# grossmanlev/FL-distributed-delay

Measured on AMD Instinct MI355X. Metric: simulated worker-steps/sec (node) @1024 workers, delay 50; aggregation HBM GB/s, higher is better.
Workload: dtype f32

## Files before the change

fl-distributed-delay_amd/csrc/common.h:

```cpp
#pragma once
#include <hip/hip_runtime.h>
#include <stdint.h>
#include <stdlib.h>

#define FLSIM_WAVE 64

#if !defined(FLSIM_LAB) &&                                                                  \
    (defined(FLSIM_X6_FRESH) || defined(FLSIM_X6_PP_V) || defined(FLSIM_DG_FMS) ||          \
     defined(FLSIM_DIRECT_FENCES) || defined(FLSIM_DX6_FENCES) || defined(FLSIM_BUFLOAD) ||  \
     defined(FLSIM_SEQ_EARLY_EXIT) || defined(FLSIM_X6_FLUSH) || defined(FLSIM_WGRAD_X6) ||     \
     defined(FLSIM_ZL1F) || defined(FLSIM_SINGLE_BUF) || defined(FLSIM_DG3_FM) || defined(FLSIM_DX_FM))
#error "FLSIM_* measurement overrides need a lab build (make LAB=1)"
#endif

typedef float f32x4 __attribute__((ext_vector_type(4)));

namespace flsim {

void set_error(const char* fmt, ...);
const char* last_error();

#define FLSIM_CHECK_HIP(expr)                                                           \
    do {                                                                                \
        hipError_t _e = (expr);                                                         \
        if (_e != hipSuccess) {                                                         \
            ::flsim::set_error("%s failed: %s (%s:%d)", #expr, hipGetErrorString(_e),   \
// ... 72 lines not shown
```

fl-distributed-delay_amd/csrc/epi_xs.h:

```cpp
#pragma once
#include "loaders.h"
#include "split.h"

namespace flsim {

__device__ __forceinline__ f32x4 mask4(f32x4 t, uint32_t pos) {
    return f32x4{(pos & 1) ? t.x : 0.f, (pos & 2) ? t.y : 0.f, (pos & 4) ? t.z : 0.f,
                 (pos & 8) ? t.w : 0.f};
}

template <int NC, int AHW>
__device__ __forceinline__ void mask_tile_sm(float* tile, int ld, const float* act, int m0, int rows,
                                             int n0, int n4, int tid, int nt) {
    const f32x2* a2 = reinterpret_cast<const f32x2*>(act);
    for (int s = 0; 4 * s < n4; ++s) {
        for (int q = tid; q < rows * 4; q += nt) {
            const int r = q >> 2, c = 4 * s + (q & 3);
            const f32x2 a = a2[2 * xs_unit<NC, AHW, true>((unsigned)(m0 + r), n0 / 4 + c)];
            f32x4* t = reinterpret_cast<f32x4*>(tile + r * ld + 4 * c);
            *t = mask4(*t, xs_pos4(a));
        }
    }
    __syncthreads();
}

template <int NC, bool SM = false, int HW = 1>
struct EpiBiasReluXs {
    static constexpr bool ASUM = false;
    static constexpr bool STAGED = true;
    static constexpr bool PARTIAL = true;
    static constexpr int NCOL = NC;
    float* Yhm;
    float* Yl;
    const float* bias;
    int M;
    float* Yf = nullptr;
    __device__ float value(int, float v) const { return v; }
    __device__ void store_rows(const float* tile, int ld, int m0, int bm, int n0, int bn, int tid,
                               int nt) const {
        const int rows = M - m0 < bm ? M - m0 : bm;
        const int n4 = bn / 4;
        for (int q = tid; q < rows * n4; q += nt) {
            const int r = q / n4, c = q - r * n4;
            const f32x4 t = *reinterpret_cast<const f32x4*>(tile + r * ld + 4 * c);
            const f32x4 b = *reinterpret_cast<const f32x4*>(bias + n0 + 4 * c);
            const f32x4 v = {fmaxf(t.x + b.x, 0.f), fmaxf(t.y + b.y, 0.f), fmaxf(t.z + b.z, 0.f),
                             fmaxf(t.w + b.w, 0.f)};
            xs_store_f(Yhm, Yl, Yf, xs_unit<NC, HW, SM>((unsigned)(m0 + r), n0 / 4 + c), v);
        }
    }
};

template <int NC, bool OUT_XS, bool ASM = false, int AHW = 1>
struct EpiMaskXs {
    static constexpr bool ASUM = false;
    static constexpr bool STAGED = true;
    static constexpr bool PARTIAL = true;
    static constexpr int NCOL = NC;
    float* Y;
    float* Yl;
    const float* act;
    int M;
    static constexpr int BATCH = 8;
// ... 106 lines not shown
        for (int pos = 0; pos < 4; ++pos) {
            f32x4 o;
            o.x = (id & 0xffu) == (uint32_t)pos ? g.x : 0.f;
            o.y = ((id >> 8) & 0xffu) == (uint32_t)pos ? g.y : 0.f;
            o.z = ((id >> 16) & 0xffu) == (uint32_t)pos ? g.z : 0.f;
            o.w = (id >> 24) == (uint32_t)pos ? g.w : 0.f;
            const long u = u0 + ((pos >> 1) * (2 * PW) + (pos & 1)) * (long)N4;
            if constexpr (OUT_XS)
                xs_store(dZhm, dZl, u, o);
            else
                st_nt4(dZhm + 4 * u, o);
        }
    }
};

template <int PH, int PW, int C, bool SM = false>
struct EpiPoolDropXs {
    static constexpr bool ASUM = false;
    static constexpr bool STAGED = true;
    static constexpr int NCOL = C;
    float* dhm;
    float* dl;
    uint8_t* idx;
    const float* bias;
    const WorkerRec* workers;
    uint64_t seed;
    uint32_t site, thr;
    float scale;
    int dropout;
    int M;
    float* df = nullptr;
    __device__ float value(int, float v) const { return v; }
    __device__ void store_rows(const float* tile, int ld, int m0, int bm, int tid, int nt) const {
        const int rows = M - m0 < bm ? M - m0 : bm;
        constexpr int C4 = C / 4;
        const int total = rows / 4 * C4;
        for (int u = tid; u < total; u += nt) {
            const int pl = u / C4, c = u - pl * C4;
            const f32x4 b = *reinterpret_cast<const f32x4*>(bias + 4 * c);
            f32x4 x[4];
#pragma unroll
            for (int r = 0; r < 4; ++r) {
                const f32x4 t = *reinterpret_cast<const f32x4*>(tile + (4 * pl + r) * ld + 4 * c);
                x[r] = f32x4{fmaxf(t.x + b.x, 0.f), fmaxf(t.y + b.y, 0.f), fmaxf(t.z + b.z, 0.f),
                             fmaxf(t.w + b.w, 0.f)};
            }
            const int q = (m0 >> 2) + pl;
            const int pw = q % PW;
            const int ph = (q / PW) % PH;
            const int s = q / (PW * PH);
            f32x4 out;
            uint32_t id = 0;
#pragma unroll
            for (int e = 0; e < 4; ++e) {
                float mv = x[0][e];
                int mi = 0;
#pragma unroll
                for (int r = 1; r < 4; ++r)
                    if (x[r][e] > mv) { mv = x[r][e]; mi = r; }
                float o = mv;
                if (dropout) {
                    const int w = s / SAMPLES_PER_WORKER;
// ... 17 lines not shown
```

fl-distributed-delay_amd/csrc/gemm_core.h:

```cpp
#pragma once
#include <type_traits>

#include "common.h"

namespace flsim {

constexpr int GK = 16;

__device__ __forceinline__ int kc_swz(int row) { return (4 - ((row >> 2) & 3)) & 3; }

template <int ROWS>
struct KCTile {
    static constexpr int FLOATS = ROWS * GK;
    __device__ static inline int chunk_off(int row, int chunk) {
        return row * GK + 4 * (chunk ^ kc_swz(row));
    }
};
template <int ROWS>
struct KMTile {
    static constexpr int STRIDE = ROWS + 4;
    static constexpr int DUMMY = GK * STRIDE;
    static constexpr int FLOATS = GK * STRIDE + 4;
};

// ... 57 lines not shown
    if constexpr (IsPartial<EPI>::value)
        epi.store_rows(tile, ld, m0, bm, n0, bn, tid, nt);
    else
        epi.store_rows(tile, ld, m0, bm, tid, nt);
}

template <class E, class = void>
struct HasPre : std::false_type {};
template <class E>
struct HasPre<E, std::void_t<decltype(E::PRE)>> : std::bool_constant<E::PRE> {};

template <class L, class = void>
struct WantsN0 : std::false_type {};
template <class L>
struct WantsN0<L, std::void_t<decltype(L::WANTS_N0)>> : std::bool_constant<L::WANTS_N0> {};

template <class E, class = void>
struct HasBiasRing : std::false_type {};
template <class E>
struct HasBiasRing<E, std::void_t<decltype(E::BIAS_RING)>> : std::bool_constant<E::BIAS_RING> {};

#ifndef FLSIM_SINGLE_BUF
#define FLSIM_SINGLE_BUF 2
#endif

template <int FM, int FN, int WAVES_M, int WAVES_N, class AL, class BL, class EPI>
__global__ void __launch_bounds__(64 * WAVES_M * WAVES_N)
gemm_kernel(AL al, BL bl, EPI epi, int ksteps_total, int ksteps_per_split, int tiles_m,
            int tiles_n) {
    constexpr int BM = 16 * FM * WAVES_M;
// ... 166 lines not shown
```

fl-distributed-delay_amd/csrc/gemm_direct.h:

```cpp
#pragma once
#include "loaders.h"

namespace flsim {

#ifndef FLSIM_DIRECT_FENCES
#define FLSIM_DIRECT_FENCES 1
#endif
constexpr bool DIRECT_FENCES = FLSIM_DIRECT_FENCES;

template <int IH, int IW, int CI, int PAD, int FM, bool WIN = false, int OHX = 0,
          class SRC = BufSrc>
struct Im2colDirect {
    using Unit = typename SRC::Unit;
    static constexpr int PIX = SRC::SM ? GK : CI;
    static constexpr int SLICE = SRC::SM ? IH * IW * GK : GK;
    static constexpr int OH = OHX > 0 ? OHX : IH + 2 * PAD - 2;
    static constexpr int OW = OHX > 0 ? OHX : IW + 2 * PAD - 2;
    static constexpr int PH = OH / 2, PW = OW / 2;
    static constexpr int ROWS_PER_IMG = WIN ? 4 * PH * PW : OH * OW;
    static_assert(CI % 16 == 0, "direct A needs whole 16-channel slices");

    const float* X;
    const float* XL = nullptr;
    int M;
    unsigned vb[FM];
    unsigned short tapmask[FM];
    SRC buf;

    __device__ void setup(int r0, int lane) {
        const int q = lane >> 4;
        buf.init(X, XL, (unsigned long)((M + ROWS_PER_IMG - 1) / ROWS_PER_IMG) * IH * IW * CI * 4);
#pragma unroll
        for (int f = 0; f < FM; ++f) {
            const int m = r0 + 16 * f + (lane & 15);
            long base = 0;
            int msk = 0;
            if (m < M) {
                const int nimg = m / ROWS_PER_IMG;
                const int rem = m - nimg * ROWS_PER_IMG;
                int oh, ow;
                if constexpr (WIN) {
                    const int qq = rem >> 2;
                    const int ph = qq / PW;
                    oh = 2 * ph + ((rem >> 1) & 1);
                    ow = 2 * (qq - ph * PW) + (rem & 1);
                } else {
                    oh = rem / OW;
                    ow = rem - oh * OW;
                }
                base = (long)nimg * IH * IW * CI + ((long)(oh - PAD) * IW + (ow - PAD)) * PIX +
                       4 * q;
#pragma unroll
                for (int t = 0; t < 9; ++t) {
                    const int ih = oh + t / 3 - PAD, iw = ow + t % 3 - PAD;
// ... 173 lines not shown
```

fl-distributed-delay_amd/csrc/gemm_dx6.h:

```cpp
#pragma once
#include "gemm_direct.h"
#include "gemm_x6.h"

namespace flsim {

#ifndef FLSIM_DX6_FENCES
#define FLSIM_DX6_FENCES 1
#endif
constexpr bool DX6_FENCES = FLSIM_DX6_FENCES;

template <int TR, int NT, int NPL>
struct RowsKCStageXs {
    using Unit = XsUnit;
    static constexpr int ROWS = TR;
    static constexpr bool KC = true;
    static constexpr int TOTAL = ROWS * 4;
    static constexpr int UNITS = (TOTAL + NT - 1) / NT;
    static constexpr int PLANE = KCTile<ROWS>::FLOATS;
    static constexpr int SPARE = NPL * PLANE;
    static constexpr int FLOATS = NPL * PLANE + 4;
    static_assert(NPL == 2 || NPL == 3, "");
    const float* P;
    const float* PL;
    long ld;
// ... 87 lines not shown
    __syncthreads();
    if constexpr (WAVES == 8) {
        if (wave >= 4) __builtin_amdgcn_s_setprio(1);
    }
    for (int s = 0; s < nst; ++s) {
        const float* Bs = lds + (s & 1) * STG;
        float* Bn = lds + ((s + 1) & 1) * STG;
        const int kn = (s + 1) * KB;
#pragma unroll
        for (int kk = 0; kk < KB; ++kk) {
            const int ks = s * KB + kk;
            if (kk > 0) bl.store(Bn + (kk - 1) * BFL, rb);
            bl.load(kn + kk, rb);
            ad.load(ks + DEPTH, ra[(kk + DEPTH) % R]);
            if constexpr (DX6_FENCES) __builtin_amdgcn_sched_barrier(0);
            const float* Bk = Bs + kk * BFL;
            f32x4 a0[FM], a1[FM];
#pragma unroll
            for (int i = 0; i < FM; ++i) {
                a0[i] = ra[kk % R][i].hm;
                a1[i] = xs_hl(ra[kk % R][i]);
            }
#pragma unroll
            for (int j = 0; j < FN; ++j) {
                const f32x4 x0 = read_frag<true, BN>(Bk, 16 * j, lane);
                const f32x4 x2 = read_frag<true, BN>(Bk + PLANE, 16 * j, lane);
                f32x4 x1;
                if constexpr (BFL >= 3 * PLANE)
                    x1 = read_frag<true, BN>(Bk + 2 * PLANE, 16 * j, lane);
                else
                    x1 = f32x4{x0.z, x0.w, x0.x, x0.y};
#pragma unroll
                for (int i = 0; i < FM; ++i) {
                    acc[i][j] = x6_step<x6_fresh(true)>(acc[i][j], a0[i], a1[i], x0, x1, x2);
                }
            }
            if constexpr (DX6_FENCES) __builtin_amdgcn_sched_barrier(0);
        }
        bl.store(Bn + (KB - 1) * BFL, rb);
        __syncthreads();
    }

    if constexpr (STAGED) {
        static_assert(BN == EPI::NCOL || (IsPartial<EPI>::value && EPI::NCOL % BN == 0),
                      "staged epilogue needs the full row in one block");
        constexpr int PASSES = (WAVES + WM_PASS - 1) / WM_PASS;
#pragma unroll 1
        for (int pass = 0; pass < PASSES; ++pass) {
            __syncthreads();
// ... 31 lines not shown
```

fl-distributed-delay_amd/csrc/gemm_x6.h:

```cpp
#pragma once
#include "gemm_core.h"
#include "split.h"

namespace flsim {

__device__ __forceinline__ f32x4 mfma_x32(f32x4 a, f32x4 b, f32x4 c) {
    return __builtin_amdgcn_mfma_f32_16x16x32_bf16(__builtin_bit_cast(bf16x8v, a),
                                                   __builtin_bit_cast(bf16x8v, b), c, 0, 0, 0);
}

template <bool FRESH>
__device__ __forceinline__ f32x4 x6_step(f32x4 acc, f32x4 a0, f32x4 a1, f32x4 b0, f32x4 b1,
                                         f32x4 b2) {
    if constexpr (FRESH) {
        f32x4 t = mfma_x32(a1, b2, f32x4{0.f, 0.f, 0.f, 0.f});
        t = mfma_x32(a0, b1, t);
        t = mfma_x32(a0, b0, t);
        return acc + t;
    } else {
        acc = mfma_x32(a1, b2, acc);
        acc = mfma_x32(a0, b1, acc);
        return mfma_x32(a0, b0, acc);
    }
}
// ... 155 lines not shown
    const int nb = gridDim.x;
    const int b = blockIdx.x;
    const int q = nb / 8, r = nb % 8, xcd = b % 8;
    const int L = (xcd < r ? xcd * (q + 1) : r * (q + 1) + (xcd - r) * q) + b / 8;
    const int tn = L % gy;
    const int tm = (L / gy) % gx;
    const int tz = L / (gx * gy);
    const int m0 = tm * BM;
    const int n0 = tn * BN;
    const int ks0 = tz * ksteps_per_split;
    int ks1 = ks0 + ksteps_per_split;
    if (ks1 > ksteps_total) ks1 = ksteps_total;

    al.setup(m0, tid);
    bl.setup(n0, tid);

    f32x4 acc[FM][FN];
#pragma unroll
    for (int i = 0; i < FM; ++i)
#pragma unroll
        for (int j = 0; j < FN; ++j) acc[i][j] = f32x4{0.f, 0.f, 0.f, 0.f};

    float asum = 0.f;
    f32x4 bacc[AMF ? FM : 1];
#pragma unroll
    for (int i = 0; i < (AMF ? FM : 1); ++i) bacc[i] = f32x4{0.f, 0.f, 0.f, 0.f};
    const bool bwave = AMF && tn == 0 && wn == 0;
    typename AL::Unit ra[AL::UNITS];
    typename BL::Unit rb[BL::UNITS];
    auto stage = [&](float* s) {
        al.each_unit(ra, [&](int a, int c, const auto& v, bool ok) { TA::store(s, a, c, v, ok); });
        bl.each_unit(rb, [&](int a, int c, const auto& v, bool ok) {
            TB::store(s + TA::FL, a, c, v, ok);
        });
    };

    if (ks0 < ks1) {
        al.load(ks0, ra);
        bl.load(ks0, rb);
        stage(lds);
        if (ks0 + 1 < ks1) {
            al.load(ks0 + 1, ra);
            bl.load(ks0 + 1, rb);
        }
    }
    __syncthreads();
    if constexpr (WAVES_M * WAVES_N == 8) {
        if (wave >= 4) __builtin_amdgcn_s_setprio(1);
    }
    int cur = 0;
    constexpr bool PP_KC = X6_PP_V > 0 && AL::KC && BL::KC && !X6Fresh<EPI>::value &&
                           std::is_same_v<typename AL::Unit, XsUnit> &&
                           std::is_same_v<typename BL::Unit, XsUnit>;
    constexpr bool PP = PP_KC;
    constexpr int PV = X6_PP_V, PW = X6_PP_W, PL = X6_PP_L;
    constexpr int FLUSH = AL::KC ? 0 : FLSIM_X6_FLUSH;
    f32x4 tot[FLUSH ? FM : 1][FLUSH ? FN : 1];
    f32x4 btot[FLUSH && AMF ? FM : 1];
    if constexpr (FLUSH > 0) {
#pragma unroll
        for (int i = 0; i < FM; ++i) {
#pragma unroll
            for (int j = 0; j < FN; ++j) tot[i][j] = f32x4{0.f, 0.f, 0.f, 0.f};
            if constexpr (AMF) btot[i] = f32x4{0.f, 0.f, 0.f, 0.f};
        }
    }
    auto main_loop = [&](auto with_sum) {
        constexpr bool WS = decltype(with_sum)::value;
        for (int ks = ks0; ks < ks1; ++ks) {
            if constexpr (PP) {
                stage(lds + (cur ^ 1) * BUF);
                const int kl = ks + 2 < ks1 ? ks + 2 : ks1 - 1;
                al.load(kl, ra);
                bl.load(kl, rb);
            } else if (ks + 1 < ks1) {
                stage(lds + (cur ^ 1) * BUF);
                if (ks + 2 < ks1) {
                    al.load(ks + 2, ra);
                    bl.load(ks + 2, rb);
                }
            }
            const float* A = lds + cur * BUF;
            const float* B = A + TA::FL;
            if constexpr (WS && !AMF) {
                if (tid < BM) asum += TA::colsum(A, tid);
            }
            typename TB::Frag bf[FN];
#pragma unroll
            for (int j = 0; j < FN; ++j) bf[j] = TB::frag(B, wn * 16 * FN + 16 * j, lane);
#pragma unroll
            for (int i = 0; i < FM; ++i) {
                const typename TA::Frag af = TA::frag(A, wm * 16 * FM + 16 * i, lane);
                if constexpr (WS && AMF) {
                    if constexpr (x6_fresh_bias()) {
// ... 119 lines not shown
```

fl-distributed-delay_amd/csrc/loaders.h:

```cpp
#pragma once
#include "gemm_core.h"
#include "pn1.h"
#include "split.h"

namespace flsim {

__device__ __forceinline__ f32x4 ldg4(const float* p) { return *reinterpret_cast<const f32x4*>(p); }
__device__ __forceinline__ f32x4 zero4() { return f32x4{0.f, 0.f, 0.f, 0.f}; }
__device__ __forceinline__ void st_nt4(float* p, f32x4 v) {
    __builtin_nontemporal_store(v, reinterpret_cast<f32x4*>(p));
}

__device__ __forceinline__ f32x4 ldg4_or0(const float* p, const float* , bool ok) {
    return ok ? ldg4(p) : zero4();
}

#ifndef FLSIM_BUFLOAD
#define FLSIM_BUFLOAD 1
#endif
constexpr unsigned BUF_OOB = 0xfffffff0u;
__device__ __forceinline__ __amdgpu_buffer_rsrc_t raw_rsrc(const void* base, unsigned long bytes) {
    const unsigned n = bytes < (unsigned long)BUF_OOB ? (unsigned)bytes : BUF_OOB;
    return __builtin_amdgcn_make_buffer_rsrc(const_cast<void*>(base), (short)0, (int)n, 0x00020000);
}
// ... 61 lines not shown
    static constexpr unsigned find(bool want_shift) {
        for (unsigned sh = 4; sh < 24; ++sh) {
            const unsigned m = ((1u << sh) + D - 1) / D;
            if ((unsigned long long)(R - 1) * m >= (1ull << 24) * 256ull) break;
            bool ok = true;
            for (unsigned r = 0; r < R && ok; ++r) ok = ((r * m) >> sh) == r / D;
            if (ok) return want_shift ? sh : m;
        }
        return 0;
    }
    static constexpr unsigned M = find(false), SH = find(true);
    static_assert(M != 0 && R * M < (1u << 31) && R < (1u << 24), "no 24-bit magic for this range");
    __device__ static unsigned div(unsigned r) { return __umul24(r, M) >> SH; }
};

template <int IH, int IW, int CI, int PAD, int TR, int NT, bool WIN = false, int OHX = 0,
          class SRC = BufSrc>
struct Im2colKC {
    using Unit = typename SRC::Unit;
    static_assert(!SRC::SM, "pixel-major operand");
    static constexpr int ROWS = TR;
    static constexpr bool KC = true;
    static constexpr int OH = OHX > 0 ? OHX : IH + 2 * PAD - 2;
    static constexpr int OW = OHX > 0 ? OHX : IW + 2 * PAD - 2;
    static constexpr int PH = OH / 2, PW = OW / 2;
    static constexpr int ROWS_PER_IMG = WIN ? 4 * PH * PW : OH * OW;
    static constexpr int TOTAL = ROWS * 4;
    static constexpr int UNITS = (TOTAL + NT - 1) / NT;
    static constexpr bool TAP_UNIFORM = CI % 16 == 0;
    static_assert(NT % 4 == 0, "");
    static_assert(CI == 4 || CI % 16 == 0, "");

    const float* X;
    const float* XL = nullptr;
    int M;
    long base[UNITS];
    unsigned vb[UNITS];
    short tapmask[UNITS];
    short row[UNITS];
    int q;
    SRC buf;
    static_assert(FLSIM_BUFLOAD || !SRC::SPLIT, "split operands use buffer loads");

    __device__ void setup(int m0, int tid) {
        q = tid & 3;
        if constexpr (FLSIM_BUFLOAD)
            buf.init(X, XL, (unsigned long)((M + ROWS_PER_IMG - 1) / ROWS_PER_IMG) * IH * IW * CI * 4);
#pragma unroll
        for (int j = 0; j < UNITS; ++j) {
            const int u = tid + j * NT;
            const int r = u >> 2;
            row[j] = (short)r;
            const int m = m0 + r;
            base[j] = 0;
            tapmask[j] = 0;
            if (u < TOTAL && m < M) {
                const int nimg = m / ROWS_PER_IMG;
                const int rem = m - nimg * ROWS_PER_IMG;
                int oh, ow;
                if constexpr (WIN) {
                    const int qq = rem >> 2;
                    const int ph = qq / PW;
                    oh = 2 * ph + ((rem >> 1) & 1);
                    ow = 2 * (qq - ph * PW) + (rem & 1);
                } else {
                    oh = rem / OW;
                    ow = rem - oh * OW;
                }
                base[j] = ((long)nimg * IH * IW + (long)(oh - PAD) * IW + (ow - PAD)) * CI + 4 * q;
                int msk = 0;
#pragma unroll
                for (int t = 0; t < 9; ++t) {
                    const int ih = oh + t / 3 - PAD, iw = ow + t % 3 - PAD;
// ... 474 lines not shown
    float* Y;
    const float* bias;
    int M;
    __device__ float value(int n, float v) const { return fmaxf(v + bias[n], 0.f); }
    __device__ void store_rows(const float* tile, int ld, int m0, int bm, int tid, int nt) const {
        const int rows = M - m0 < bm ? M - m0 : bm;
        constexpr int N4 = NC / 4;
        f32x4* dst = reinterpret_cast<f32x4*>(Y + (long)m0 * NC);
        for (int q = tid; q < rows * N4; q += nt) {
            const int r = q / N4, c = q - r * N4;
            st_nt4(reinterpret_cast<float*>(dst + q), *reinterpret_cast<const f32x4*>(tile + r * ld + 4 * c));
        }
    }
};

template <int PH, int PW, int C, bool NCHW_OUT>
struct EpiPoolDrop {
    static constexpr bool ASUM = false;
    float* d;
    uint8_t* idx;
    const float* bias;
    const WorkerRec* workers;
    uint64_t seed;
    uint32_t site, thr;
    float scale;
    int dropout;
    int M;
    __device__ void apply4(int m, int n, int z, f32x4 v) const {
        if (n >= C || m >= M) return;
        const float b = bias[n];
        float mv = fmaxf(v[0] + b, 0.f);
        int mi = 0;
#pragma unroll
        for (int r = 1; r < 4; ++r) {
            const float x = fmaxf(v[r] + b, 0.f);
            if (x > mv) { mv = x; mi = r; }
        }
        const int q = m >> 2;
        const int pw = q % PW;
        const int ph = (q / PW) % PH;
        const int s = q / (PW * PH);
        const int w = s / SAMPLES_PER_WORKER;
        const int nl = s - w * SAMPLES_PER_WORKER;
        float out = mv;
        if (dropout) {
            const WorkerRec wr = workers[w];
            const uint32_t en = (uint32_t)(((nl * C + n) * PH + ph) * PW + pw);
            out = philox_word(seed, wr.t, wr.i, site, en) >= thr ? mv * scale : 0.f;
        }
        const long e = (long)q * C + n;
        idx[e] = (uint8_t)mi;
        if (NCHW_OUT)
            d[(long)s * (C * PH * PW) + (n * PH + ph) * PW + pw] = out;
// ... 221 lines not shown
```

fl-distributed-delay_amd/csrc/net_kernels.h:

```cpp
#pragma once
#include "epi_xs.h"
#include "gemm_direct.h"
#include "gemm_dx6.h"
#include "gemm_x6.h"
#include "loaders.h"
#include "pn1.h"
#include "probe.h"

namespace flsim {

static __global__ void __launch_bounds__(256)
k_fill_batch(const uint8_t* __restrict__ pool, const int32_t* __restrict__ labels,
             const int32_t* __restrict__ list_a, int len_a, const int32_t* __restrict__ list_b,
             int len_b, const WorkerRec* __restrict__ workers, int n_workers_total, uint64_t seed,
             const float* __restrict__ lut, float* __restrict__ x0, int32_t* __restrict__ y) {
    const int s = blockIdx.x;
    const int w = s / SAMPLES_PER_WORKER;
    const int j = s - w * SAMPLES_PER_WORKER;
    const WorkerRec wr = workers[w];
    const uint32_t bsz = wr.pad ? wr.pad : (uint32_t)SAMPLES_PER_WORKER;
    const uint32_t q = (wr.i >> 20) * SAMPLES_PER_WORKER + (uint32_t)j;
    float* out = x0 + (long)s * 4096;
    if (q >= bsz) {
        if (threadIdx.x == 0) y[s] = -1;
// ... 827 lines not shown
}

template <int IH, int IW, int CI, int PAD, int FM, int FN, int WM, int WN, int FMS, int FNS,
          int WMS, int WNS, int VO = 0, bool DZC = false, bool X6 = false, class SRC = BufSrc,
          class SRCB = SRC>
static int conv_wgrad_sz(const float* dz, const float* X, int S, int CO, int KP, float* slab,
                         float* bslab, int Z, hipStream_t st, int kid, int kreal, int zinit,
                         int* zused, const float* dzl = nullptr, const float* Xl = nullptr) {
    if (S <= small_chunk_samples())
        return conv_wgrad<IH, IW, CI, PAD, FMS, FNS, WMS, WNS, VO, DZC, X6, SRC, SRCB>(
            dz, X, S, CO, KP, slab, bslab, Z, st, kid, kreal, zinit, zused, dzl, Xl);
    return conv_wgrad<IH, IW, CI, PAD, FM, FN, WM, WN, VO, DZC, X6, SRC, SRCB>(
        dz, X, S, CO, KP, slab, bslab, Z, st, kid, kreal, zinit, zused, dzl, Xl);
}

template <int IH, int IW, int CI, int PAD, int FM, int FN, int WAVES, int KB, int DEPTH, int NPL,
          bool WIN, int OHX, class ASRC = XsSrc, class EPI>
static int conv_dx6(XsT X, int S, XsT W, int N, int KP, const EPI& epi, hipStream_t st, int kid,
                    int kreal) {
    static_assert(ASRC::SPLIT, "split input");
    using AD = Im2colDirect<IH, IW, CI, PAD, FM, WIN, OHX, ASRC>;
    using BL = RowsKCStageXs<16 * FN, 64 * WAVES, NPL>;
    constexpr int BM = 16 * FM * WAVES, BN = 16 * FN;
    FLSIM_REQUIRE((KP / GK) % KB == 0, "direct GEMM: %d k-steps not a multiple of %d", KP / GK, KB);
    AD ad;
    ad.X = X.hm;
    ad.XL = X.l;
    ad.M = S * AD::ROWS_PER_IMG;
    BL bl;
    bl.P = W.hm;
    bl.PL = W.l;
    bl.ld = KP;
    bl.NR = N;
    const int tm = ceil_div(ad.M, BM), tn = ceil_div(N, BN);
    const ProbeSlot ps = probe_begin();
    hipExtLaunchKernelGGL((gemm_dx6_kernel<FM, FN, WAVES, KB, DEPTH, AD, BL, EPI>),
                          dim3(tm * tn), dim3(64 * WAVES), 0, st, ps.start, ps.stop, 0, ad, bl,
                          epi, KP / GK, tm, tn);
    FLSIM_LAUNCH_CHECK();
    return probe_end(ps, kid, 2.0 * ad.M * N * kreal);
}

template <int IH, int IW, int CI, int PAD, int FM, int FN, int WM, int WN, bool WIN, int OHX,
          class EPI>
static int conv_xs(XsT X, int S, XsT W, int N, int KP, const EPI& epi, hipStream_t st, int kid,
                   int kreal) {
    constexpr int NT = 64 * WM * WN;
    constexpr int BM = 16 * FM * WM, BN = 16 * FN * WN;
    using AL = Im2colKC<IH, IW, CI, PAD, BM, NT, WIN, OHX, XsSrc>;
    using BL = RowsKC<BN, NT, XsSrc>;
    AL al;
    al.X = X.hm;
    al.XL = X.l;
    al.M = S * AL::ROWS_PER_IMG;
    BL bl;
    bl.P = W.hm;
    bl.PL = W.l;
    bl.ld = KP;
    bl.NR = N;
    return launch_gemm<FM, FN, WM, WN, true>(al, bl, epi, al.M, N, KP / GK, 1, st, kid,
                                             2.0 * al.M * N * kreal);
}

template <int IH, int IW, int CI, int CO, int PAD, int FM, int FN, int WM, int WN, bool NCHW_OUT,
          bool X6 = false>
static int conv_pool_fwd(const float* X, int S, const float* Wpk, int KP, float* d, uint8_t* idx,
                         const float* bias, const WorkerRec* workers, uint64_t seed, uint32_t site,
                         uint32_t thr, float scale, int dropout, hipStream_t st, int kid,
                         int kreal) {
    constexpr int NT = 64 * WM * WN;
    constexpr int BM = 16 * FM * WM, BN = 16 * FN * WN;
    using AL = Im2colKC<IH, IW, CI, PAD, BM, NT, true>;
    using BL = RowsKC<BN, NT>;
    AL al;
    al.X = X;
    al.M = S * AL::ROWS_PER_IMG;
// ... 55 lines not shown
```

fl-distributed-delay_amd/csrc/pn1_net.hip:

```cpp
#include <stdarg.h>
#include <stdio.h>
#include <string.h>

#include <mutex>
#include <unordered_map>

#include "net_abi.h"

namespace flsim {

static thread_local char g_err[512];
void set_error(const char* fmt, ...) {
    va_list ap;
    va_start(ap, fmt);
    vsnprintf(g_err, sizeof(g_err), fmt, ap);
    va_end(ap);
}
const char* last_error() { return g_err; }

struct ConvGeo {
    int CI, CIP, CO, H;
    int KP;
    int ZW;
};
// ... 231 lines not shown
    const long units = M / C1_ROWS;
    const int grid = (int)(units / 4 < 2048 ? (units + 3) / 4 : 2048);
    const ProbeSlot ps = probe_begin();
    hipExtLaunchKernelGGL(k_conv1_fwd, dim3(grid), dim3(256), 0, st, ps.start, ps.stop, 0, x0, W,
                          bias, a1.hm, a1.l, a1f, units);
    FLSIM_LAUNCH_CHECK();
    return probe_end(ps, K_FWD1, 2.0 * M * 48 * 27);
}

#ifndef FLSIM_DX_FM
#define FLSIM_DX_FM 4
#endif
constexpr int DX_FM = FLSIM_DX_FM, DX_FMS = 1, DX_KB = 3, DX_DEPTH = 2, DX_NPL = 2;


template <int IH, int IW, int CI, int PAD, int FN, bool WIN, int OHX, int FM = DX_FM,
          int WAVES = 8, int FMS = (FM == DX_FM ? DX_FMS : FM / 2), class EPI>
static int dx6(XsT X, int S, XsT W, int N, int KP, const EPI& epi, hipStream_t st, int kid,
               int kreal) {
    if (S <= small_chunk_samples())
        return conv_dx6<IH, IW, CI, PAD, FMS, FN, WAVES, DX_KB, DX_DEPTH, DX_NPL, WIN, OHX,
                        XsSrcSM>(X, S, W, N, KP, epi, st, kid, kreal);
    return conv_dx6<IH, IW, CI, PAD, FM, FN, WAVES, DX_KB, DX_DEPTH, DX_NPL, WIN, OHX, XsSrcSM>(
        X, S, W, N, KP, epi, st, kid, kreal);
}

template <int IH, int IW, int CI, int PAD, int FM, int FN, int WM, int WN, bool WIN, int OHX,
          class EPI>
static int xs(XsT X, int S, XsT W, int N, int KP, const EPI& epi, hipStream_t st, int kid,
              int kreal) {
    if (S <= small_chunk_samples())
        return conv_xs<IH, IW, CI, PAD, FM / 2, FN, WM, WN, WIN, OHX>(X, S, W, N, KP, epi, st, kid,
                                                                     kreal);
    return conv_xs<IH, IW, CI, PAD, FM, FN, WM, WN, WIN, OHX>(X, S, W, N, KP, epi, st, kid, kreal);
}

static int forward(const GradState& g, const WS& w, const float* theta, int S,
                   const WorkerRec* workers, uint64_t seed, int dropout, hipStream_t st) {
    const XsT a1 = w.x(w.a1, w.a1l), d1 = w.x(w.d1, w.d1l), a3 = w.x(w.a3, w.a3l);
    const XsT d2 = w.x(w.d2, w.d2l), a5 = w.x(w.a5, w.a5l);
    RC(conv1_fwd(w.x0, theta + P_OFF[0], theta + P_OFF[1], a1, w.a1f, S, st));
    RC((dx6<34, 34, 48, 2, 3, true, 0, 4, 4, 2>(a1, S, g.wfx[1], 48, 432,
        EpiPoolDropXs<18, 18, 48, true>{d1.hm, d1.l, w.i1, theta + P_OFF[3], workers, seed, SITE_DROP1,
                                  THR_P25, SCALE_P25, dropout, S * 18 * 18 * 4, w.d1f}, st,
        K_FWD2, 432)));
    RC((dx6<18, 18, 48, 2, 6, false, 0>(d1, S, g.wfx[2], 96, 432,
        EpiBiasReluXs<96, true, 400>{a3.hm, a3.l, theta + P_OFF[5], S * 20 * 20, w.a3f}, st, K_FWD3,
        432)));
    RC((dx6<20, 20, 96, 2, 6, true, 0>(a3, S, g.wfx[3], 96, 864,
        EpiPoolDropXs<11, 11, 96>{d2.hm, d2.l, w.i2, theta + P_OFF[7], workers, seed, SITE_DROP2,
                                  THR_P25, SCALE_P25, dropout, S * 11 * 11 * 4, w.d2f}, st,
        K_FWD4, 864)));
    RC((xs<11, 11, 96, 2, 4, 6, 4, 2, false, 0>(d2, S, g.wfx[4], 192, 864,
        EpiBiasReluXs<192>{a5.hm, a5.l, theta + P_OFF[9], S * 13 * 13, w.a5f}, st, K_FWD5, 864)));
    RC((xs<13, 13, 192, 2, 4, 6, 4, 2, true, 0>(a5, S, g.wfx[5], 192, 1728,
        EpiPoolDrop<7, 7, 192, true>{w.d3, w.i3, theta + P_OFF[11], workers, seed, SITE_DROP3,
                                     THR_P25, SCALE_P25, dropout, S * 7 * 7 * 4}, st, K_FWD6,
        1728)));
    if (S <= 2048)
        RC((linear_fwd<1, 2, 2, 2, true, EpiSlabStoreFresh>(w.d3, theta + P_OFF[12], w.part, S,
                                                            512, 9408, ZL1F, st, K_L1F)));
    else if (S <= 4096)
        RC((linear_fwd<2, 2, 2, 2, true, EpiSlabStoreFresh>(w.d3, theta + P_OFF[12], w.part, S,
                                                            512, 9408, ZL1F, st, K_L1F)));
    else
        RC((linear_fwd<4, 4, 2, 2, true, EpiSlabStoreFresh>(w.d3, theta + P_OFF[12], w.part, S,
                                                            512, 9408, ZL1F, st, K_L1F)));
    RC(linear_finish(w.part, ZL1F, theta + P_OFF[13], w.e1, S, 512, workers, seed, SITE_DROP4,
                     THR_P50, SCALE_P50, dropout, st));
    RC((linear_fwd<2, 2, 2, 2>(w.e1, theta + P_OFF[14], w.part, S, 256, 512, 1, st, K_L2F)));
    RC(linear_finish(w.part, 1, theta + P_OFF[15], w.e2, S, 256, workers, seed, SITE_DROP5,
                     THR_P50, SCALE_P50, dropout, st));
    return 0;
// ... 565 lines not shown
```

Baseline: 1173.

## Reorder conv GEMM rows image-minor to skip out-of-bounds padding taps

Adds an image-minor row mapping (RowMap) so each GEMM tile or wave covers the same output pixel across a group of images. That makes the set of in-bounds 3x3 taps uniform per tile, and the k-loop can skip padding taps entirely: remapped k-steps in the x6 GEMM, predicated steps in dx6. Only the fifth forward conv layer enables it by default; the other layers get compile-time switches. Epilogues remap rows back to image-major order. The cost is extra index arithmetic, a padded M extent rounded up to whole groups, and a per-tile varying k-loop length that can unbalance work across tiles.

```diff
diff --git a/fl-distributed-delay_amd/csrc/common.h b/fl-distributed-delay_amd/csrc/common.h
--- a/fl-distributed-delay_amd/csrc/common.h
+++ b/fl-distributed-delay_amd/csrc/common.h
@@ -9,7 +9,9 @@
     (defined(FLSIM_X6_FRESH) || defined(FLSIM_X6_PP_V) || defined(FLSIM_DG_FMS) ||          \
      defined(FLSIM_DIRECT_FENCES) || defined(FLSIM_DX6_FENCES) || defined(FLSIM_BUFLOAD) ||  \
      defined(FLSIM_SEQ_EARLY_EXIT) || defined(FLSIM_X6_FLUSH) || defined(FLSIM_WGRAD_X6) ||     \
-     defined(FLSIM_ZL1F) || defined(FLSIM_SINGLE_BUF) || defined(FLSIM_DG3_FM) || defined(FLSIM_DX_FM))
+     defined(FLSIM_ZL1F) || defined(FLSIM_SINGLE_BUF) || defined(FLSIM_DG3_FM) || defined(FLSIM_DX_FM) || \
+     defined(FLSIM_FWD_IM2) || defined(FLSIM_FWD_IM3) || defined(FLSIM_FWD_IM4) ||            \
+     defined(FLSIM_FWD_IM5) || defined(FLSIM_FWD_IM6))
 #error "FLSIM_* measurement overrides need a lab build (make LAB=1)"
 #endif
 
diff --git a/fl-distributed-delay_amd/csrc/epi_xs.h b/fl-distributed-delay_amd/csrc/epi_xs.h
--- a/fl-distributed-delay_amd/csrc/epi_xs.h
+++ b/fl-distributed-delay_amd/csrc/epi_xs.h
@@ -24,7 +24,7 @@
     __syncthreads();
 }
 
-template <int NC, bool SM = false, int HW = 1>
+template <int NC, bool SM = false, int HW = 1, int GRP = 0>
 struct EpiBiasReluXs {
     static constexpr bool ASUM = false;
     static constexpr bool STAGED = true;
@@ -38,15 +38,22 @@
     __device__ float value(int, float v) const { return v; }
     __device__ void store_rows(const float* tile, int ld, int m0, int bm, int n0, int bn, int tid,
                                int nt) const {
-        const int rows = M - m0 < bm ? M - m0 : bm;
+        const int rows = GRP > 0 || M - m0 >= bm ? bm : M - m0;
         const int n4 = bn / 4;
         for (int q = tid; q < rows * n4; q += nt) {
             const int r = q / n4, c = q - r * n4;
+            unsigned m = (unsigned)(m0 + r);
+            if constexpr (GRP > 0) {
+                unsigned img, pix;
+                RowMap<GRP, HW>::split(m, img, pix);
+                if (img >= (unsigned)(M / HW)) continue;
+                m = img * (unsigned)HW + pix;
+            }
             const f32x4 t = *reinterpret_cast<const f32x4*>(tile + r * ld + 4 * c);
             const f32x4 b = *reinterpret_cast<const f32x4*>(bias + n0 + 4 * c);
             const f32x4 v = {fmaxf(t.x + b.x, 0.f), fmaxf(t.y + b.y, 0.f), fmaxf(t.z + b.z, 0.f),
                              fmaxf(t.w + b.w, 0.f)};
-            xs_store_f(Yhm, Yl, Yf, xs_unit<NC, HW, SM>((unsigned)(m0 + r), n0 / 4 + c), v);
+            xs_store_f(Yhm, Yl, Yf, xs_unit<NC, HW, SM>(m, n0 / 4 + c), v);
         }
     }
 };
@@ -183,7 +190,7 @@
     }
 };
 
-template <int PH, int PW, int C, bool SM = false>
+template <int PH, int PW, int C, bool SM = false, int GRP = 0>
 struct EpiPoolDropXs {
     static constexpr bool ASUM = false;
     static constexpr bool STAGED = true;
@@ -201,11 +208,18 @@
     float* df = nullptr;
     __device__ float value(int, float v) const { return v; }
     __device__ void store_rows(const float* tile, int ld, int m0, int bm, int tid, int nt) const {
-        const int rows = M - m0 < bm ? M - m0 : bm;
+        const int rows = GRP > 0 || M - m0 >= bm ? bm : M - m0;
         constexpr int C4 = C / 4;
         const int total = rows / 4 * C4;
         for (int u = tid; u < total; u += nt) {
             const int pl = u / C4, c = u - pl * C4;
+            int q = (m0 >> 2) + pl;
+            if constexpr (GRP > 0) {
+                unsigned img, win;
+                RowMap<GRP, PH * PW>::split((unsigned)q, img, win);
+                if (img >= (unsigned)(M / (4 * PH * PW))) continue;
+                q = (int)(img * (unsigned)(PH * PW) + win);
+            }
             const f32x4 b = *reinterpret_cast<const f32x4*>(bias + 4 * c);
             f32x4 x[4];
 #pragma unroll
@@ -214,7 +228,6 @@
                 x[r] = f32x4{fmaxf(t.x + b.x, 0.f), fmaxf(t.y + b.y, 0.f), fmaxf(t.z + b.z, 0.f),
                              fmaxf(t.w + b.w, 0.f)};
             }
-            const int q = (m0 >> 2) + pl;
             const int pw = q % PW;
             const int ph = (q / PW) % PH;
             const int s = q / (PW * PH);
diff --git a/fl-distributed-delay_amd/csrc/gemm_core.h b/fl-distributed-delay_amd/csrc/gemm_core.h
--- a/fl-distributed-delay_amd/csrc/gemm_core.h
+++ b/fl-distributed-delay_amd/csrc/gemm_core.h
@@ -95,6 +95,11 @@
 struct WantsN0 : std::false_type {};
 template <class L>
 struct WantsN0<L, std::void_t<decltype(L::WANTS_N0)>> : std::bool_constant<L::WANTS_N0> {};
+
+template <class L, class = void>
+struct TapSkip : std::false_type {};
+template <class L>
+struct TapSkip<L, std::void_t<decltype(L::TAP_SKIP)>> : std::bool_constant<L::TAP_SKIP> {};
 
 template <class E, class = void>
 struct HasBiasRing : std::false_type {};
diff --git a/fl-distributed-delay_amd/csrc/gemm_direct.h b/fl-distributed-delay_amd/csrc/gemm_direct.h
--- a/fl-distributed-delay_amd/csrc/gemm_direct.h
+++ b/fl-distributed-delay_amd/csrc/gemm_direct.h
@@ -9,9 +9,12 @@
 constexpr bool DIRECT_FENCES = FLSIM_DIRECT_FENCES;
 
 template <int IH, int IW, int CI, int PAD, int FM, bool WIN = false, int OHX = 0,
-          class SRC = BufSrc>
+          class SRC = BufSrc, int GRP = 0>
 struct Im2colDirect {
     using Unit = typename SRC::Unit;
+    static constexpr bool TAP_SKIP = GRP > 0;
+    static_assert(GRP == 0 || GRP == (WIN ? 4 * FM : 16 * FM),
+                  "image-minor rows: one pixel (window) per wave");
     static constexpr int PIX = SRC::SM ? GK : CI;
     static constexpr int SLICE = SRC::SM ? IH * IW * GK : GK;
     static constexpr int OH = OHX > 0 ? OHX : IH + 2 * PAD - 2;
@@ -25,19 +28,33 @@
     int M;
     unsigned vb[FM];
     unsigned short tapmask[FM];
+    int wtaps;
     SRC buf;
+    static constexpr int UNITS_PER_IMG = WIN ? PH * PW : OH * OW;
+    using Map = RowMap<GRP, UNITS_PER_IMG>;
+
+    __device__ bool live(int ks) const { return (wtaps >> (ks % 9)) & 1; }
+    __host__ __device__ static constexpr int unit_live_taps(int unit) {
+        return unit_taps<IH, IW, PAD, OW, PW, WIN>(unit);
+    }
 
     __device__ void setup(int r0, int lane) {
         const int q = lane >> 4;
         buf.init(X, XL, (unsigned long)((M + ROWS_PER_IMG - 1) / ROWS_PER_IMG) * IH * IW * CI * 4);
+        if constexpr (TAP_SKIP) {
+            const int unit = __builtin_amdgcn_readfirstlane(r0 / (16 * FM)) % UNITS_PER_IMG;
+            wtaps = unit_live_taps(unit);
+        }
+        const int S = M / ROWS_PER_IMG;
 #pragma unroll
         for (int f = 0; f < FM; ++f) {
             const int m = r0 + 16 * f + (lane & 15);
             long base = 0;
             int msk = 0;
-            if (m < M) {
-                const int nimg = m / ROWS_PER_IMG;
-                const int rem = m - nimg * ROWS_PER_IMG;
+            unsigned nimg, unit;
+            Map::split((unsigned)(WIN ? m >> 2 : m), nimg, unit);
+            if (GRP > 0 ? nimg < (unsigned)S : m < M) {
+                const int rem = WIN ? 4 * (int)unit + (m & 3) : (int)unit;
                 int oh, ow;
                 if constexpr (WIN) {
                     const int qq = rem >> 2;
diff --git a/fl-distributed-delay_amd/csrc/gemm_dx6.h b/fl-distributed-delay_amd/csrc/gemm_dx6.h
--- a/fl-distributed-delay_amd/csrc/gemm_dx6.h
+++ b/fl-distributed-delay_amd/csrc/gemm_dx6.h
@@ -125,25 +125,29 @@
             bl.load(kn + kk, rb);
             ad.load(ks + DEPTH, ra[(kk + DEPTH) % R]);
             if constexpr (DX6_FENCES) __builtin_amdgcn_sched_barrier(0);
-            const float* Bk = Bs + kk * BFL;
-            f32x4 a0[FM], a1[FM];
-#pragma unroll
-            for (int i = 0; i < FM; ++i) {
-                a0[i] = ra[kk % R][i].hm;
-                a1[i] = xs_hl(ra[kk % R][i]);
-            }
-#pragma unroll
-            for (int j = 0; j < FN; ++j) {
-                const f32x4 x0 = read_frag<true, BN>(Bk, 16 * j, lane);
-                const f32x4 x2 = read_frag<true, BN>(Bk + PLANE, 16 * j, lane);
-                f32x4 x1;
-                if constexpr (BFL >= 3 * PLANE)
-                    x1 = read_frag<true, BN>(Bk + 2 * PLANE, 16 * j, lane);
-                else
-                    x1 = f32x4{x0.z, x0.w, x0.x, x0.y};
+            bool run = true;
+            if constexpr (TapSkip<AD>::value) run = ad.live(ks);
+            if (run) {
+                const float* Bk = Bs + kk * BFL;
+                f32x4 a0[FM], a1[FM];
 #pragma unroll
                 for (int i = 0; i < FM; ++i) {
-                    acc[i][j] = x6_step<x6_fresh(true)>(acc[i][j], a0[i], a1[i], x0, x1, x2);
+                    a0[i] = ra[kk % R][i].hm;
+                    a1[i] = xs_hl(ra[kk % R][i]);
+                }
+#pragma unroll
+                for (int j = 0; j < FN; ++j) {
+                    const f32x4 x0 = read_frag<true, BN>(Bk, 16 * j, lane);
+                    const f32x4 x2 = read_frag<true, BN>(Bk + PLANE, 16 * j, lane);
+                    f32x4 x1;
+                    if constexpr (BFL >= 3 * PLANE)
+                        x1 = read_frag<true, BN>(Bk + 2 * PLANE, 16 * j, lane);
+                    else
+                        x1 = f32x4{x0.z, x0.w, x0.x, x0.y};
+#pragma unroll
+                    for (int i = 0; i < FM; ++i) {
+                        acc[i][j] = x6_step<x6_fresh(true)>(acc[i][j], a0[i], a1[i], x0, x1, x2);
+                    }
                 }
             }
             if constexpr (DX6_FENCES) __builtin_amdgcn_sched_barrier(0);
diff --git a/fl-distributed-delay_amd/csrc/gemm_x6.h b/fl-distributed-delay_amd/csrc/gemm_x6.h
--- a/fl-distributed-delay_amd/csrc/gemm_x6.h
+++ b/fl-distributed-delay_amd/csrc/gemm_x6.h
@@ -193,6 +193,12 @@
 
     al.setup(m0, tid);
     bl.setup(n0, tid);
+    constexpr bool SKIP = TapSkip<AL>::value;
+    if constexpr (SKIP) ks1 = ks0 + al.live_ksteps(ks1 - ks0);
+    auto kreal = [&](int kc) {
+        if constexpr (SKIP) return al.kmap(kc);
+        else return kc;
+    };
 
     f32x4 acc[FM][FN];
 #pragma unroll
@@ -215,12 +221,12 @@
     };
 
     if (ks0 < ks1) {
-        al.load(ks0, ra);
-        bl.load(ks0, rb);
+        al.load(kreal(ks0), ra);
+        bl.load(kreal(ks0), rb);
         stage(lds);
         if (ks0 + 1 < ks1) {
-            al.load(ks0 + 1, ra);
-            bl.load(ks0 + 1, rb);
+            al.load(kreal(ks0 + 1), ra);
+            bl.load(kreal(ks0 + 1), rb);
         }
     }
     __syncthreads();
@@ -249,14 +255,14 @@
         for (int ks = ks0; ks < ks1; ++ks) {
             if constexpr (PP) {
                 stage(lds + (cur ^ 1) * BUF);
-                const int kl = ks + 2 < ks1 ? ks + 2 : ks1 - 1;
+                const int kl = kreal(ks + 2 < ks1 ? ks + 2 : ks1 - 1);
                 al.load(kl, ra);
                 bl.load(kl, rb);
             } else if (ks + 1 < ks1) {
                 stage(lds + (cur ^ 1) * BUF);
                 if (ks + 2 < ks1) {
-                    al.load(ks + 2, ra);
-                    bl.load(ks + 2, rb);
+                    al.load(kreal(ks + 2), ra);
+                    bl.load(kreal(ks + 2), rb);
                 }
             }
             const float* A = lds + cur * BUF;
diff --git a/fl-distributed-delay_amd/csrc/loaders.h b/fl-distributed-delay_amd/csrc/loaders.h
--- a/fl-distributed-delay_amd/csrc/loaders.h
+++ b/fl-distributed-delay_amd/csrc/loaders.h
@@ -99,8 +99,49 @@
     __device__ static unsigned div(unsigned r) { return __umul24(r, M) >> SH; }
 };
 
+template <int G, int U>
+struct RowMap {
+    static_assert(G >= 0 && (G & (G - 1)) == 0, "group size: a power of two");
+    __host__ __device__ static constexpr long units(int S) {
+        return G == 0 ? (long)S * U : (long)((S + G - 1) / (G > 0 ? G : 1)) * G * U;
+    }
+    __device__ static void split(unsigned u, unsigned& img, unsigned& unit) {
+        if constexpr (G == 0) {
+            img = u / (unsigned)U;
+            unit = u - img * (unsigned)U;
+        } else {
+            const unsigned gu = u / (unsigned)G, j = u - gu * (unsigned)G;
+            const unsigned grp = gu / (unsigned)U;
+            unit = gu - grp * (unsigned)U;
+            img = grp * (unsigned)G + j;
+        }
+    }
+};
+
+template <int IH, int IW, int PAD>
+__host__ __device__ constexpr int taps_of(int oh, int ow) {
+    int msk = 0;
+    for (int t = 0; t < 9; ++t) {
+        const int ih = oh + t / 3 - PAD, iw = ow + t % 3 - PAD;
+        if ((unsigned)ih < (unsigned)IH && (unsigned)iw < (unsigned)IW) msk |= 1 << t;
+    }
+    return msk;
+}
+template <int IH, int IW, int PAD, int OW, int PW, bool WIN>
+__host__ __device__ constexpr int unit_taps(int unit) {
+    if constexpr (WIN) {
+        const int ph = unit / PW, pw = unit - ph * PW;
+        return taps_of<IH, IW, PAD>(2 * ph, 2 * pw) | taps_of<IH, IW, PAD>(2 * ph, 2 * pw + 1) |
+               taps_of<IH, IW, PAD>(2 * ph + 1, 2 * pw) |
+               taps_of<IH, IW, PAD>(2 * ph + 1, 2 * pw + 1);
+    } else {
+        const int oh = unit / OW;
+        return taps_of<IH, IW, PAD>(oh, unit - oh * OW);
+    }
+}
+
 template <int IH, int IW, int CI, int PAD, int TR, int NT, bool WIN = false, int OHX = 0,
-          class SRC = BufSrc>
+          class SRC = BufSrc, int GRP = 0>
 struct Im2colKC {
     using Unit = typename SRC::Unit;
     static_assert(!SRC::SM, "pixel-major operand");
@@ -110,6 +151,11 @@
     static constexpr int OW = OHX > 0 ? OHX : IW + 2 * PAD - 2;
     static constexpr int PH = OH / 2, PW = OW / 2;
     static constexpr int ROWS_PER_IMG = WIN ? 4 * PH * PW : OH * OW;
+    static constexpr int UNITS_PER_IMG = WIN ? PH * PW : OH * OW;
+    using Map = RowMap<GRP, UNITS_PER_IMG>;
+    static constexpr bool TAP_SKIP = GRP > 0;
+    static_assert(GRP == 0 || (GRP == (WIN ? TR / 4 : TR) && CI % 16 == 0),
+                  "image-minor rows: one pixel (window) per tile");
     static constexpr int TOTAL = ROWS * 4;
     static constexpr int UNITS = (TOTAL + NT - 1) / NT;
     static constexpr bool TAP_UNIFORM = CI % 16 == 0;
@@ -125,12 +171,35 @@
     short row[UNITS];
     int q;
     SRC buf;
+    unsigned long taplist;
+    int ntaps;
+    unsigned tinv;
     static_assert(FLSIM_BUFLOAD || !SRC::SPLIT, "split operands use buffer loads");
+
+    __host__ __device__ static constexpr int unit_live_taps(int unit) {
+        return unit_taps<IH, IW, PAD, OW, PW, WIN>(unit);
+    }
+    __device__ int live_ksteps(int total) const { return total / 9 * ntaps; }
+    __device__ int kmap(int kc) const {
+        const int cs = (int)(((unsigned)kc * tinv) >> 16);
+        return 9 * cs + (int)((taplist >> (4 * (kc - cs * ntaps))) & 15);
+    }
 
     __device__ void setup(int m0, int tid) {
         q = tid & 3;
         if constexpr (FLSIM_BUFLOAD)
             buf.init(X, XL, (unsigned long)((M + ROWS_PER_IMG - 1) / ROWS_PER_IMG) * IH * IW * CI * 4);
+        if constexpr (TAP_SKIP) {
+            const int unit = (m0 / TR) % UNITS_PER_IMG;
+            const int live = unit_live_taps(unit);
+            taplist = 0;
+            ntaps = 0;
+#pragma unroll
+            for (int t = 0; t < 9; ++t)
+                if ((live >> t) & 1) taplist |= (unsigned long)t << (4 * ntaps++);
+            tinv = (65536u + ntaps - 1) / (unsigned)ntaps;
+        }
+        const int S = M / ROWS_PER_IMG;
 #pragma unroll
         for (int j = 0; j < UNITS; ++j) {
             const int u = tid + j * NT;
@@ -139,9 +208,10 @@
             const int m = m0 + r;
             base[j] = 0;
             tapmask[j] = 0;
-            if (u < TOTAL && m < M) {
-                const int nimg = m / ROWS_PER_IMG;
-                const int rem = m - nimg * ROWS_PER_IMG;
+            unsigned nimg, unit;
+            Map::split((unsigned)(WIN ? m >> 2 : m), nimg, unit);
+            if (u < TOTAL && (GRP > 0 ? nimg < (unsigned)S : m < M)) {
+                const int rem = WIN ? 4 * (int)unit + (m & 3) : (int)unit;
                 int oh, ow;
                 if constexpr (WIN) {
                     const int qq = rem >> 2;
@@ -646,7 +716,7 @@
     }
 };
 
-template <int PH, int PW, int C, bool NCHW_OUT>
+template <int PH, int PW, int C, bool NCHW_OUT, int GRP = 0>
 struct EpiPoolDrop {
     static constexpr bool ASUM = false;
     float* d;
@@ -659,7 +729,14 @@
     int dropout;
     int M;
     __device__ void apply4(int m, int n, int z, f32x4 v) const {
-        if (n >= C || m >= M) return;
+        if (n >= C || (GRP == 0 && m >= M)) return;
+        int q = m >> 2;
+        if constexpr (GRP > 0) {
+            unsigned img, win;
+            RowMap<GRP, PH * PW>::split((unsigned)q, img, win);
+            if (img >= (unsigned)(M / (4 * PH * PW))) return;
+            q = (int)(img * (unsigned)(PH * PW) + win);
+        }
         const float b = bias[n];
         float mv = fmaxf(v[0] + b, 0.f);
         int mi = 0;
@@ -668,7 +745,6 @@
             const float x = fmaxf(v[r] + b, 0.f);
             if (x > mv) { mv = x; mi = r; }
         }
-        const int q = m >> 2;
         const int pw = q % PW;
         const int ph = (q / PW) % PH;
         const int s = q / (PW * PH);
diff --git a/fl-distributed-delay_amd/csrc/net_kernels.h b/fl-distributed-delay_amd/csrc/net_kernels.h
--- a/fl-distributed-delay_amd/csrc/net_kernels.h
+++ b/fl-distributed-delay_amd/csrc/net_kernels.h
@@ -865,12 +865,25 @@
         dz, X, S, CO, KP, slab, bslab, Z, st, kid, kreal, zinit, zused, dzl, Xl);
 }
 
+template <class AL, int GRP>
+static double conv_flops(int S, int N, int kreal) {
+    if constexpr (GRP == 0) {
+        return 2.0 * ((double)S * AL::ROWS_PER_IMG) * N * kreal;
+    } else {
+        long pairs = 0;
+        for (int u = 0; u < AL::UNITS_PER_IMG; ++u)
+            pairs += __builtin_popcount(AL::unit_live_taps(u));
+        pairs *= AL::ROWS_PER_IMG / AL::UNITS_PER_IMG;
+        return 2.0 * (double)S * (double)pairs * N * (kreal / 9.0);
+    }
+}
+
 template <int IH, int IW, int CI, int PAD, int FM, int FN, int WAVES, int KB, int DEPTH, int NPL,
-          bool WIN, int OHX, class ASRC = XsSrc, class EPI>
+          bool WIN, int OHX, class ASRC = XsSrc, int GRP = 0, class EPI>
 static int conv_dx6(XsT X, int S, XsT W, int N, int KP, const EPI& epi, hipStream_t st, int kid,
                     int kreal) {
     static_assert(ASRC::SPLIT, "split input");
-    using AD = Im2colDirect<IH, IW, CI, PAD, FM, WIN, OHX, ASRC>;
+    using AD = Im2colDirect<IH, IW, CI, PAD, FM, WIN, OHX, ASRC, GRP>;
     using BL = RowsKCStageXs<16 * FN, 64 * WAVES, NPL>;
     constexpr int BM = 16 * FM * WAVES, BN = 16 * FN;
     FLSIM_REQUIRE((KP / GK) % KB == 0, "direct GEMM: %d k-steps not a multiple of %d", KP / GK, KB);
@@ -883,22 +896,23 @@
     bl.PL = W.l;
     bl.ld = KP;
     bl.NR = N;
-    const int tm = ceil_div(ad.M, BM), tn = ceil_div(N, BN);
+    const long rows = AD::Map::units(S) * (WIN ? 4 : 1);
+    const int tm = (int)ceil_div(rows, (long)BM), tn = ceil_div(N, BN);
     const ProbeSlot ps = probe_begin();
     hipExtLaunchKernelGGL((gemm_dx6_kernel<FM, FN, WAVES, KB, DEPTH, AD, BL, EPI>),
                           dim3(tm * tn), dim3(64 * WAVES), 0, st, ps.start, ps.stop, 0, ad, bl,
                           epi, KP / GK, tm, tn);
     FLSIM_LAUNCH_CHECK();
-    return probe_end(ps, kid, 2.0 * ad.M * N * kreal);
+    return probe_end(ps, kid, conv_flops<AD, GRP>(S, N, kreal));
 }
 
 template <int IH, int IW, int CI, int PAD, int FM, int FN, int WM, int WN, bool WIN, int OHX,
-          class EPI>
+          int GRP = 0, class EPI>
 static int conv_xs(XsT X, int S, XsT W, int N, int KP, const EPI& epi, hipStream_t st, int kid,
                    int kreal) {
     constexpr int NT = 64 * WM * WN;
     constexpr int BM = 16 * FM * WM, BN = 16 * FN * WN;
-    using AL = Im2colKC<IH, IW, CI, PAD, BM, NT, WIN, OHX, XsSrc>;
+    using AL = Im2colKC<IH, IW, CI, PAD, BM, NT, WIN, OHX, XsSrc, GRP>;
     using BL = RowsKC<BN, NT, XsSrc>;
     AL al;
     al.X = X.hm;
@@ -909,8 +923,9 @@
     bl.PL = W.l;
     bl.ld = KP;
     bl.NR = N;
-    return launch_gemm<FM, FN, WM, WN, true>(al, bl, epi, al.M, N, KP / GK, 1, st, kid,
-                                             2.0 * al.M * N * kreal);
+    const long rows = AL::Map::units(S) * (WIN ? 4 : 1);
+    return launch_gemm<FM, FN, WM, WN, true>(al, bl, epi, (int)rows, N, KP / GK, 1, st, kid,
+                                             conv_flops<AL, GRP>(S, N, kreal));
 }
 
 template <int IH, int IW, int CI, int CO, int PAD, int FM, int FN, int WM, int WN, bool NCHW_OUT,
diff --git a/fl-distributed-delay_amd/csrc/pn1_net.hip b/fl-distributed-delay_amd/csrc/pn1_net.hip
--- a/fl-distributed-delay_amd/csrc/pn1_net.hip
+++ b/fl-distributed-delay_amd/csrc/pn1_net.hip
@@ -269,25 +269,45 @@
 constexpr int DX_FM = FLSIM_DX_FM, DX_FMS = 1, DX_KB = 3, DX_DEPTH = 2, DX_NPL = 2;
 
 
+#ifndef FLSIM_FWD_IM2
+#define FLSIM_FWD_IM2 0
+#endif
+#ifndef FLSIM_FWD_IM3
+#define FLSIM_FWD_IM3 0
+#endif
+#ifndef FLSIM_FWD_IM4
+#define FLSIM_FWD_IM4 0
+#endif
+#ifndef FLSIM_FWD_IM5
+#define FLSIM_FWD_IM5 1
+#endif
+#ifndef FLSIM_FWD_IM6
+#define FLSIM_FWD_IM6 0
+#endif
+
 template <int IH, int IW, int CI, int PAD, int FN, bool WIN, int OHX, int FM = DX_FM,
-          int WAVES = 8, int FMS = (FM == DX_FM ? DX_FMS : FM / 2), class EPI>
-static int dx6(XsT X, int S, XsT W, int N, int KP, const EPI& epi, hipStream_t st, int kid,
+          int WAVES = 8, int FMS = (FM == DX_FM ? DX_FMS : FM / 2), bool IM = false, class MK>
+static int dx6(XsT X, int S, XsT W, int N, int KP, const MK& mk, hipStream_t st, int kid,
                int kreal) {
+    constexpr int GL = IM ? (WIN ? 4 : 16) * FM : 0, GS = IM ? (WIN ? 4 : 16) * FMS : 0;
     if (S <= small_chunk_samples())
         return conv_dx6<IH, IW, CI, PAD, FMS, FN, WAVES, DX_KB, DX_DEPTH, DX_NPL, WIN, OHX,
-                        XsSrcSM>(X, S, W, N, KP, epi, st, kid, kreal);
-    return conv_dx6<IH, IW, CI, PAD, FM, FN, WAVES, DX_KB, DX_DEPTH, DX_NPL, WIN, OHX, XsSrcSM>(
-        X, S, W, N, KP, epi, st, kid, kreal);
+                        XsSrcSM, GS>(X, S, W, N, KP, mk(std::integral_constant<int, GS>{}), st,
+                                     kid, kreal);
+    return conv_dx6<IH, IW, CI, PAD, FM, FN, WAVES, DX_KB, DX_DEPTH, DX_NPL, WIN, OHX, XsSrcSM,
+                    GL>(X, S, W, N, KP, mk(std::integral_constant<int, GL>{}), st, kid, kreal);
 }
 
 template <int IH, int IW, int CI, int PAD, int FM, int FN, int WM, int WN, bool WIN, int OHX,
-          class EPI>
-static int xs(XsT X, int S, XsT W, int N, int KP, const EPI& epi, hipStream_t st, int kid,
+          bool IM = false, class MK>
+static int xs(XsT X, int S, XsT W, int N, int KP, const MK& mk, hipStream_t st, int kid,
               int kreal) {
+    constexpr int GL = IM ? (WIN ? 4 : 16) * FM * WM : 0, GS = GL / 2;
     if (S <= small_chunk_samples())
-        return conv_xs<IH, IW, CI, PAD, FM / 2, FN, WM, WN, WIN, OHX>(X, S, W, N, KP, epi, st, kid,
-                                                                     kreal);
-    return conv_xs<IH, IW, CI, PAD, FM, FN, WM, WN, WIN, OHX>(X, S, W, N, KP, epi, st, kid, kreal);
+        return conv_xs<IH, IW, CI, PAD, FM / 2, FN, WM, WN, WIN, OHX, GS>(
+            X, S, W, N, KP, mk(std::integral_constant<int, GS>{}), st, kid, kreal);
+    return conv_xs<IH, IW, CI, PAD, FM, FN, WM, WN, WIN, OHX, GL>(
+        X, S, W, N, KP, mk(std::integral_constant<int, GL>{}), st, kid, kreal);
 }
 
 static int forward(const GradState& g, const WS& w, const float* theta, int S,
@@ -295,23 +315,34 @@
     const XsT a1 = w.x(w.a1, w.a1l), d1 = w.x(w.d1, w.d1l), a3 = w.x(w.a3, w.a3l);
     const XsT d2 = w.x(w.d2, w.d2l), a5 = w.x(w.a5, w.a5l);
     RC(conv1_fwd(w.x0, theta + P_OFF[0], theta + P_OFF[1], a1, w.a1f, S, st));
-    RC((dx6<34, 34, 48, 2, 3, true, 0, 4, 4, 2>(a1, S, g.wfx[1], 48, 432,
-        EpiPoolDropXs<18, 18, 48, true>{d1.hm, d1.l, w.i1, theta + P_OFF[3], workers, seed, SITE_DROP1,
-                                  THR_P25, SCALE_P25, dropout, S * 18 * 18 * 4, w.d1f}, st,
-        K_FWD2, 432)));
-    RC((dx6<18, 18, 48, 2, 6, false, 0>(d1, S, g.wfx[2], 96, 432,
-        EpiBiasReluXs<96, true, 400>{a3.hm, a3.l, theta + P_OFF[5], S * 20 * 20, w.a3f}, st, K_FWD3,
-        432)));
-    RC((dx6<20, 20, 96, 2, 6, true, 0>(a3, S, g.wfx[3], 96, 864,
-        EpiPoolDropXs<11, 11, 96>{d2.hm, d2.l, w.i2, theta + P_OFF[7], workers, seed, SITE_DROP2,
-                                  THR_P25, SCALE_P25, dropout, S * 11 * 11 * 4, w.d2f}, st,
-        K_FWD4, 864)));
-    RC((xs<11, 11, 96, 2, 4, 6, 4, 2, false, 0>(d2, S, g.wfx[4], 192, 864,
-        EpiBiasReluXs<192>{a5.hm, a5.l, theta + P_OFF[9], S * 13 * 13, w.a5f}, st, K_FWD5, 864)));
-    RC((xs<13, 13, 192, 2, 4, 6, 4, 2, true, 0>(a5, S, g.wfx[5], 192, 1728,
-        EpiPoolDrop<7, 7, 192, true>{w.d3, w.i3, theta + P_OFF[11], workers, seed, SITE_DROP3,
-                                     THR_P25, SCALE_P25, dropout, S * 7 * 7 * 4}, st, K_FWD6,
-        1728)));
+    RC((dx6<34, 34, 48, 2, 3, true, 0, 4, 4, 2, FLSIM_FWD_IM2>(a1, S, g.wfx[1], 48, 432,
+        [&](auto G) {
+            return EpiPoolDropXs<18, 18, 48, true, decltype(G)::value>{
+                d1.hm, d1.l, w.i1, theta + P_OFF[3], workers, seed, SITE_DROP1, THR_P25,
+                SCALE_P25, dropout, S * 18 * 18 * 4, w.d1f};
+        }, st, K_FWD2, 432)));
+    RC((dx6<18, 18, 48, 2, 6, false, 0, DX_FM, 8, DX_FMS, FLSIM_FWD_IM3>(d1, S, g.wfx[2], 96, 432,
+        [&](auto G) {
+            return EpiBiasReluXs<96, true, 400, decltype(G)::value>{
+                a3.hm, a3.l, theta + P_OFF[5], S * 20 * 20, w.a3f};
+        }, st, K_FWD3, 432)));
+    RC((dx6<20, 20, 96, 2, 6, true, 0, DX_FM, 8, DX_FMS, FLSIM_FWD_IM4>(a3, S, g.wfx[3], 96, 864,
+        [&](auto G) {
+            return EpiPoolDropXs<11, 11, 96, false, decltype(G)::value>{
+                d2.hm, d2.l, w.i2, theta + P_OFF[7], workers, seed, SITE_DROP2, THR_P25,
+                SCALE_P25, dropout, S * 11 * 11 * 4, w.d2f};
+        }, st, K_FWD4, 864)));
+    RC((xs<11, 11, 96, 2, 4, 6, 4, 2, false, 0, FLSIM_FWD_IM5>(d2, S, g.wfx[4], 192, 864,
+        [&](auto G) {
+            return EpiBiasReluXs<192, false, 169, decltype(G)::value>{
+                a5.hm, a5.l, theta + P_OFF[9], S * 13 * 13, w.a5f};
+        }, st, K_FWD5, 864)));
+    RC((xs<13, 13, 192, 2, 4, 6, 4, 2, true, 0, FLSIM_FWD_IM6>(a5, S, g.wfx[5], 192, 1728,
+        [&](auto G) {
+            return EpiPoolDrop<7, 7, 192, true, decltype(G)::value>{
+                w.d3, w.i3, theta + P_OFF[11], workers, seed, SITE_DROP3, THR_P25, SCALE_P25,
+                dropout, S * 7 * 7 * 4};
+        }, st, K_FWD6, 1728)));
     if (S <= 2048)
         RC((linear_fwd<1, 2, 2, 2, true, EpiSlabStoreFresh>(w.d3, theta + P_OFF[12], w.part, S,
                                                             512, 9408, ZL1F, st, K_L1F)));
```

Result: no change. 1181, median of 6 (+0.6%).
